# nlesc-dirac/sagecal

Hardware: NVIDIA H100
Metric: baseline_visibilities_per_sec_predict_jacobian (higher is better)
Workload: dtype f64

## Files before the change

sagecal_b200/csrc/lm.cu:

```cuda
#include <float.h>
#include <math.h>
#include <string.h>
#include <vector>

#include "../../include/dirac_b200.h"
#include "problem.h"

#define CS_CHECK(call)                                                                     \
  do {                                                                                     \
    cusolverStatus_t s__ = (call);                                                         \
    if (s__ != CUSOLVER_STATUS_SUCCESS) {                                                  \
      fprintf(stderr, "dirac_b200: cuSOLVER error %d at %s:%d\n", (int)s__, __FILE__, __LINE__); \
      exit(1);                                                                             \
    }                                                                                      \
  } while (0)
#define CB_CHECK(call)                                                                     \
  do {                                                                                     \
    cublasStatus_t s__ = (call);                                                           \
    if (s__ != CUBLAS_STATUS_SUCCESS) {                                                    \
      fprintf(stderr, "dirac_b200: cuBLAS error %d at %s:%d\n", (int)s__, __FILE__, __LINE__); \
      exit(1);                                                                             \
    }                                                                                      \
  } while (0)

extern "C" {
void db_launch_weighted_jtj(const WeightedJtjArgs *a, int ntile, cudaStream_t st);
void db_launch_sum_abs(const double2 *v, long long R, long long r0, long long r1, double *partials,
                       double *out, unsigned int *counter, cudaStream_t st);
void db_launch_update_weights(const double2 *e, double2 *wt, long long R, long long r0,
                              long long r1, double nu0, double *partials, double *out,
                              unsigned int *counter, cudaStream_t st);
void db_launch_scale_vis(double2 *v, long long R, long long r0, long long r1, double alpha,
                         int set_const, cudaStream_t st);
void db_launch_extract_diag(const double *A, double *dst, int n, cudaStream_t st);
void db_launch_lm_step(const double *p, const double *Dp, const double *jte, double *pnew,
                       double *sc, double *zero, int n, cudaStream_t st);
void db_launch_os_shift(const double2 *e, const double2 *wt, double2 *eps, double2 *wout, long long R,
                        long long row_sub0, long long nrow_sub, long long row_chunk0, long long kl,
                        long long nJ, cudaStream_t st);
}

template <typename T>
static T *dalloc(size_t n) {
  return (T *)db_malloc(n * sizeof(T) + 16);
}

void db_lm_init(dirac_b200_problem *pr) {
  LMWork &w = pr->lm;
  if (w.ready) return;
  DevProblem &d = pr->d;
  const int n8 = 8 * d.N;
  w.n8 = n8;
  w.T = dalloc<double>((size_t)d.Mt * d.Nbase * 16);
  w.T_valid = (unsigned char *)calloc(d.Mt, 1);
  w.Tsub = dalloc<double>((size_t)d.Nbase * 16);
  w.JTJ0 = dalloc<double>((size_t)n8 * n8);
  w.JTJ = dalloc<double>((size_t)n8 * n8);
  w.JTe = d.scal + 64 + n8;
  w.JTe_new = d.scal + 64 + 2 * n8;
  w.Hst = dalloc<double>((size_t)4 * d.N);
  w.Dp = d.scal + 64;
  w.pnew = dalloc<double>(n8);
  w.plast = dalloc<double>(n8);
  w.pold = dalloc<double>(n8);
  w.devinfo = reinterpret_cast<int *>(d.scal + 64 + 3 * n8);
  w.tau = dalloc<double>(n8);
  w.svdS = w.svdU = w.svdVT = nullptr;
  w.wbuf = w.ebuf = nullptr;
  w.os_eps = w.os_w = nullptr;
  w.HP = w.HQ = nullptr;
  w.JB = w.LB = nullptr;
  w.sys_T = w.sys_p = w.sys_H = nullptr;
  w.pref_slot = (int *)malloc(sizeof(int) * d.M);
  for (int k = 0; k < d.M; k++) w.pref_slot[k] = -1;
  w.jtj0_cur = nullptr;
  w.jtj_spec = nullptr;
  {
    const int nbg = (d.Nbase + 255) / 256;
    const int nsl = db_cp_max_slices(d.Nbase, d.tilesz);
    w.jte_part = dalloc<double>((size_t)nbg * (nsl + 1) * n8);
  }
  DB_CHECK(cudaEventCreateWithFlags(&w.ev_mail, cudaEventDisableTiming));
  DB_CHECK(cudaMallocHost((void **)&w.h_vec, sizeof(double) * (5 * n8 + 4 * d.N + 64)));
  static cusolverDnHandle_t g_cs = nullptr;
  static cublasHandle_t g_cb = nullptr;
  if (!g_cs) {
    CS_CHECK(cusolverDnCreate(&g_cs));
    CB_CHECK(cublasCreate(&g_cb));
  }
  w.cs = g_cs;
  w.cb = g_cb;
  CS_CHECK(cusolverDnSetStream(w.cs, d.stream));
  CB_CHECK(cublasSetStream(w.cb, d.stream));
  int l1 = 0, l2 = 0, l3 = 0;
  CS_CHECK(cusolverDnDpotrf_bufferSize(w.cs, CUBLAS_FILL_MODE_LOWER, n8, w.JTJ, n8, &l1));
  CS_CHECK(cusolverDnDgeqrf_bufferSize(w.cs, n8, n8, w.JTJ, n8, &l2));
  CS_CHECK(cusolverDnDormqr_bufferSize(w.cs, CUBLAS_SIDE_LEFT, CUBLAS_OP_T, n8, 1, n8, w.JTJ, n8,
                                       w.tau, w.Dp, n8, &l3));
  w.lwork = l1 > l2 ? l1 : l2;
  if (l3 > w.lwork) w.lwork = l3;
  int l4 = 0;
  CS_CHECK(cusolverDnDgesvd_bufferSize(w.cs, n8, n8, &l4));
  if (l4 > w.lwork) w.lwork = l4;
  w.own_chol = n8 <= db_chol_max_n() && db_chol_available() && !getenv("DIRAC_B200_CUSOLVER");
  if (w.own_chol && (size_t)w.lwork < db_chol_ws_doubles(n8)) w.lwork = (int)db_chol_ws_doubles(n8);
  w.cswork = dalloc<double>((size_t)w.lwork);
  w.bt_ws = nullptr;
  w.bt_epoch = 0;
  if (!w.own_chol && db_bigtri_available(n8)) {
    const size_t nd = db_bigtri_ws_doubles(n8);
    w.bt_ws = dalloc<double>(nd);
    DB_CHECK(cudaMemsetAsync(w.bt_ws, 0, sizeof(double) * nd, d.stream));
  }
  w.dbuf = dalloc<double2>((size_t)4 * d.R);
  w.ready = true;
}

static void robust_init(dirac_b200_problem *pr) {
  LMWork &w = pr->lm;
  if (w.wbuf) return;
  DevProblem &d = pr->d;
  w.wbuf = dalloc<double2>((size_t)4 * d.R);
  w.ebuf = dalloc<double2>((size_t)4 * d.R);
  w.HP = dalloc<double>((size_t)d.N * 20);
  w.HQ = dalloc<double>((size_t)d.N * 20);
}

static void os_init(dirac_b200_problem *pr) {
  robust_init(pr);
  LMWork &w = pr->lm;
  if (w.os_eps) return;
  w.os_eps = dalloc<double2>((size_t)4 * pr->d.R);
  w.os_w = dalloc<double2>((size_t)4 * pr->d.R);
}

void db_lm_free(dirac_b200_problem *pr) {
  LMWork &w = pr->lm;
  if (!w.ready) return;
  db_free(w.T); db_free(w.Tsub); db_free(w.JTJ0); db_free(w.JTJ);
  db_free(w.Hst); db_free(w.pnew); db_free(w.plast); db_free(w.pold); db_free(w.jte_part);
  db_free(w.tau); db_free(w.cswork); db_free(w.dbuf);
  if (w.bt_ws) db_free(w.bt_ws);
  if (w.svdS) { db_free(w.svdS); db_free(w.svdU); db_free(w.svdVT); }
  if (w.wbuf) { db_free(w.wbuf); db_free(w.ebuf); db_free(w.HP); db_free(w.HQ); }
  if (w.os_eps) { db_free(w.os_eps); db_free(w.os_w); }
  if (w.LB) {
    if (w.JB) db_free(w.JB);
    db_free(w.LB); db_free(w.HB); db_free(w.mu_dev); db_free(w.binfo_dev);
    db_free(w.LBptr_dev); db_free(w.blist_dev); db_free(w.btix_dev); db_free(w.bpoff_dev);
    cudaFreeHost(w.h_mu); cudaFreeHost(w.h_binfo);
  }
  free(w.pref_slot);
  cudaEventDestroy(w.ev_mail);
  cudaFreeHost(w.h_vec);
  free(w.T_valid);
  w.ready = false;
}

static int pick_tslice(const DevProblem &d, int nt) {
  int target_ctas = db_sm_count();
  int slices = (target_ctas + d.ntile - 1) / d.ntile;
  if (slices < 1) slices = 1;
  int ts = (nt + slices - 1) / slices;
  if (ts < 2) ts = 2;
  if (ts > nt) ts = nt;
  if (ts < 1) ts = 1;
  return ts;
}

void db_cluster_pass(dirac_b200_problem *pr, int k, const double *pblk_dev, const double2 *in,
                     double2 *out, int mode, int write_out, double *jte_dev, int cost_slot, int t0,
                     int t1, const double2 *wt, double beta = 1.0, const double2 *in2 = nullptr,
                     bool jte_zeroed = false, const double *pblk_old = nullptr,
                     bool form_hidden = false);

void db_cluster_pass(dirac_b200_problem *pr, int k, const double *pblk_dev, const double2 *in,
                     double2 *out, int mode, int write_out, double *jte_dev, int cost_slot, int t0,
                     int t1, const double2 *wt, double beta, const double2 *in2, bool jte_zeroed,
                     const double *pblk_old, bool form_hidden) {
  DevProblem &d = pr->d;
  if (t1 <= t0) {
    if (mode <= 1 || mode == 4)
      DB_CHECK(cudaMemsetAsync(d.scal + cost_slot, 0, sizeof(double), d.stream));
    if (jte_dev) DB_CHECK(cudaMemsetAsync(jte_dev, 0, sizeof(double) * 8 * d.N, d.stream));
    return;
  }
  ClusterPassArgs a;
  a.coh_k = d.coh + (size_t)k * 4 * d.R;
  a.in = in; a.flag = d.flag; a.pblk = pblk_dev; a.tiles = d.tiles; a.out = out; a.jte = jte_dev;
  a.blpq = d.blpq; a.jte_part = pr->lm.jte_part; a.gcounter = d.counters + 16;
  a.partials = pr->partials; a.cost = d.scal + cost_slot; a.counter = d.counters; a.R = d.R;
  a.N = d.N; a.Nbase = d.Nbase; a.t_begin = t0; a.t_end = t1; a.tslice = pick_tslice(d, t1 - t0);
  a.mode = mode; a.write_out = write_out; a.wt = wt; a.beta = beta; a.in2 = in2;
  a.pblk_old = pblk_old; a.form_hidden = form_hidden;
  if (!(jte_dev && (mode <= 1 || mode == 4)) && a.tslice > 1)
    a.tslice = (a.tslice + 1) / 2;
  if (jte_dev && (mode <= 1 || mode == 4) && !jte_zeroed)
    DB_CHECK(cudaMemsetAsync(jte_dev, 0, sizeof(double) * 8 * d.N, d.stream));
  db_prof_begin((jte_dev && (mode <= 1 || mode == 4)) ? 2 : 8, (double)(t1 - t0) * d.Nbase * (129.0 + (write_out ? 64.0 : 0.0) +
                                                 (wt ? 64.0 : 0.0)), d.stream);
  db_launch_cluster_pass(&a, d.ntile, d.stream);
  db_prof_end(d.stream);
  db_count_launch(1);
}

static void gram(dirac_b200_problem *pr, int k, int t0, int t1, int step, double *Tdst) {
  DevProblem &d = pr->d;
  GramArgs a;
  a.coh = d.coh; a.flag = d.flag; a.tiles = d.tiles; a.T = Tdst; a.R = d.R; a.N = d.N;
  a.Nbase = d.Nbase; a.k0 = k; a.t_begin = t0; a.t_end = t1; a.t_step = step;
  db_prof_begin(3, (double)((t1 - t0 + step - 1) / step) * d.Nbase * 65.0 + 128.0 * d.Nbase,
                d.stream);
  db_launch_coh_gram(&a, d.ntile, 1, d.stream);
  db_prof_end(d.stream);
  db_count_launch(1);
}

static AssembleArgs assemble_args(const DevProblem &d, const double *T, const double *pblk_dev,
                                  double *Hst) {
  AssembleArgs a;
  memset(&a, 0, sizeof(a));
  a.T = T; a.pblk = pblk_dev; a.Hst = Hst; a.N = d.N; a.Nbase = d.Nbase;
  return a;
}

static void station_sums(dirac_b200_problem *pr, const AssembleArgs &a, int nb) {
  DevProblem &d = pr->d;
  db_prof_begin(4, nb * 256.0 * d.Nbase, d.stream);
  db_launch_station_sums(&a, nb, d.stream);
  db_prof_end(d.stream);
  db_count_launch(1);
}

static void assemble_tiles(dirac_b200_problem *pr, const AssembleArgs &a, int nb) {
  DevProblem &d = pr->d;
  const double n = 8.0 * d.N;
  db_prof_begin(4, nb * (a.lower ? 128.0 * d.Nbase + 4.0 * n * (n + 1) : 256.0 * d.Nbase + 8.0 * n * n),
                d.stream);
  db_launch_assemble_tiles(&a, nb, d.stream);
  db_prof_end(d.stream);
  db_count_launch(1);
}

static void assemble(dirac_b200_problem *pr, const double *T, const double *pblk_dev,
                     double *JTJ) {
  AssembleArgs a = assemble_args(pr->d, T, pblk_dev, pr->lm.Hst);
  station_sums(pr, a, 1);
  if (!JTJ) return;
  a.JTJ = JTJ;
  assemble_tiles(pr, a, 1);
}

static void weighted_jtj(dirac_b200_problem *pr, int k, int t0, int t1, const double *pblk_dev,
                         const double2 *wt, double *JTJ) {
  DevProblem &d = pr->d;
  LMWork &w = pr->lm;
  const int n = w.n8;
  DB_CHECK(cudaMemsetAsync(JTJ, 0, sizeof(double) * (size_t)n * n, d.stream));
  DB_CHECK(cudaMemsetAsync(w.HP, 0, sizeof(double) * 20 * d.N, d.stream));
  DB_CHECK(cudaMemsetAsync(w.HQ, 0, sizeof(double) * 20 * d.N, d.stream));
  if (t1 <= t0) return;
  WeightedJtjArgs a;
  a.coh_k = d.coh + (size_t)k * 4 * d.R;
  a.wt = wt; a.flag = d.flag; a.pblk = pblk_dev; a.tiles = d.tiles; a.JTJ = JTJ; a.HP = w.HP;
  a.HQ = w.HQ; a.R = d.R; a.N = d.N; a.Nbase = d.Nbase; a.t_begin = t0; a.t_end = t1;
  a.tslice = pick_tslice(d, t1 - t0);
  db_prof_begin(6, (double)(t1 - t0) * d.Nbase * 129.0 + 8.0 * 64.0 * d.N * d.N, d.stream);
  db_launch_weighted_jtj(&a, d.ntile, d.stream);
  db_prof_end(d.stream);
  db_count_launch(2);
}

void db_chunk_range(const DevProblem &d, int k, int ck, int *t0, int *t1);
static void chunk_range(const DevProblem &d, int k, int ck, int *t0, int *t1) {
  db_chunk_range(d, k, ck, t0, t1);
}
void db_chunk_range(const DevProblem &d, int k, int ck, int *t0, int *t1) {
  int nchunk = d.h_clus[k].nchunk;
  int tilechunk = (d.tilesz + nchunk - 1) / nchunk;
  int a = ck * tilechunk;
  int b = a + tilechunk;
  if (a > d.tilesz) a = d.tilesz;
  if (b > d.tilesz) b = d.tilesz;
  *t0 = a;
  *t1 = b;
}

static int enqueue_solve(dirac_b200_problem *pr, double mu, int linsolv, double eps1) {
  DevProblem &d = pr->d;
  LMWork &w = pr->lm;
  const int n = w.n8;
  int *hinfo = (int *)(w.h_vec + 4 * n + 4 * d.N);
  hinfo[0] = hinfo[1] = 0;
  if (linsolv == 0 && w.own_chol) {
    db_prof_begin(5, 0.0, d.stream);
    db_launch_chol_solve(w.jtj0_cur ? w.jtj0_cur : w.JTJ0, n, mu, w.JTe, w.Dp, w.cswork, w.devinfo,
                         d.stream);
    db_prof_end(d.stream);
    db_count_launch(1);
    w.step_fused = w.step_armed;
    return 1;
  }
  if (linsolv == 0 && w.sys_T) {
    AssembleArgs a = assemble_args(d, w.sys_T, w.sys_p, const_cast<double *>(w.sys_H));
    a.JTJ = w.JTJ;
    a.mu = mu;
    a.lower = 1;
    assemble_tiles(pr, a, 1);
  } else {
    db_prof_begin(4, 16.0 * n * n, d.stream);
    db_launch_copy_add_diag(w.jtj0_cur ? w.jtj0_cur : w.JTJ0, w.JTJ, n, mu, d.stream);
    db_prof_end(d.stream);
    db_count_launch(1);
  }
  DB_CHECK(cudaMemcpyAsync(w.Dp, w.JTe, sizeof(double) * n, cudaMemcpyDeviceToDevice, d.stream));
  db_prof_begin(5, 0.0, d.stream);
  if (linsolv == 0) {
    CS_CHECK(cusolverDnDpotrf(w.cs, CUBLAS_FILL_MODE_LOWER, n, w.JTJ, n, w.cswork, w.lwork,
                              w.devinfo));
    if (w.bt_ws) {
      DB_CHECK(cudaMemsetAsync(w.devinfo + 1, 0, sizeof(int), d.stream));
      db_launch_bigtri_solve(w.JTJ, n, n, w.JTe, w.Dp, w.bt_ws, ++w.bt_epoch, 1, d.stream);
      db_count_launch(4);
    } else {
      CS_CHECK(cusolverDnDpotrs(w.cs, CUBLAS_FILL_MODE_LOWER, n, 1, w.JTJ, n, w.Dp, n,
                                w.devinfo + 1));
      db_count_launch(2);
    }
  } else if (linsolv == 1) {
    CS_CHECK(cusolverDnDgeqrf(w.cs, n, n, w.JTJ, n, w.tau, w.cswork, w.lwork, w.devinfo));
    CS_CHECK(cusolverDnDormqr(w.cs, CUBLAS_SIDE_LEFT, CUBLAS_OP_T, n, 1, n, w.JTJ, n, w.tau, w.Dp,
                              n, w.cswork, w.lwork, w.devinfo + 1));
    const double one = 1.0;
    CB_CHECK(cublasDtrsm(w.cb, CUBLAS_SIDE_LEFT, CUBLAS_FILL_MODE_UPPER, CUBLAS_OP_N,
                         CUBLAS_DIAG_NON_UNIT, n, 1, &one, w.JTJ, n, w.Dp, n));
    db_count_launch(3);
  } else {
    if (!w.svdS) {
      w.svdS = dalloc<double>(n);
      w.svdU = dalloc<double>((size_t)n * n);
      w.svdVT = dalloc<double>((size_t)n * n);
    }
    CS_CHECK(cusolverDnDgesvd(w.cs, 'A', 'A', n, n, w.JTJ, n, w.svdS, w.svdU, n, w.svdVT, n,
                              w.cswork, w.lwork, nullptr, w.devinfo));
    db_count_launch(1);
    double *hS = (double *)malloc(sizeof(double) * n);
    double *hb = (double *)malloc(sizeof(double) * n);
    const double one = 1.0, zero = 0.0;
    CB_CHECK(cublasDgemv(w.cb, CUBLAS_OP_T, n, n, &one, w.svdU, n, w.JTe, 1, &zero, w.Dp, 1));
    DB_CHECK(cudaMemcpyAsync(hS, w.svdS, sizeof(double) * n, cudaMemcpyDeviceToHost, d.stream));
    DB_CHECK(cudaMemcpyAsync(hb, w.Dp, sizeof(double) * n, cudaMemcpyDeviceToHost, d.stream));
    db_stream_sync(d.stream);
    for (int i = 0; i < n; i++) hb[i] = (hS[i] > eps1) ? hb[i] / hS[i] : 0.0;
    DB_CHECK(cudaMemcpyAsync(w.pnew, hb, sizeof(double) * n, cudaMemcpyHostToDevice, d.stream));
    CB_CHECK(cublasDgemv(w.cb, CUBLAS_OP_T, n, n, &one, w.svdVT, n, w.pnew, 1, &zero, w.Dp, 1));
    db_prof_end(d.stream);
    DB_CHECK(cudaMemcpyAsync(w.h_vec + 2 * n, w.Dp, sizeof(double) * n, cudaMemcpyDeviceToHost,
                             d.stream));
    db_stream_sync(d.stream);
    free(hS);
    free(hb);
    db_count_launch(2);
    return 1;
  }
  db_prof_end(d.stream);
  (void)hinfo;
  return 1;
}

static double nrm2sq(const double *v, int n) {
  double s = 0.0;
  for (int i = 0; i < n; i++) s += v[i] * v[i];
  return s;
}

void db_prefactor_sweep(dirac_b200_problem *pr, double tau) {
  DevProblem &d = pr->d;
  db_lm_init(pr);
  LMWork &w = pr->lm;
  const int n = w.n8;
  const size_t nn = (size_t)n * n;
  const bool own_batch = w.own_chol && db_tri_available(n) && !getenv("DIRAC_B200_BATCH_CUSOLVER");
  const bool keep_jb = w.own_chol;
  if ((double)d.M * nn * 8.0 * (keep_jb ? 2 : 1) > 24e9) return;
  const size_t lstride = own_batch ? db_chol_ws_doubles(n) : nn;
  w.lb_stride = lstride;
  w.lb_ld = own_batch ? 32 * ((n + 31) / 32) : n;
  if (!w.LB) {
    w.JB = keep_jb ? dalloc<double>(nn * d.M) : nullptr;
    w.LB = dalloc<double>(lstride * d.M);
    w.HB = dalloc<double>((size_t)4 * d.N * d.M);
    w.mu_dev = dalloc<double>(d.M);
    w.binfo_dev = dalloc<int>(2 * d.M);
    w.LBptr_dev = (double **)dalloc<double *>(d.M);
    w.blist_dev = dalloc<int>(d.M);
    w.btix_dev = dalloc<int>(d.M);
    w.bpoff_dev = dalloc<int>(d.M);
    DB_CHECK(cudaMallocHost((void **)&w.h_mu, sizeof(double) * d.M));
    DB_CHECK(cudaMallocHost((void **)&w.h_binfo, sizeof(int) * 2 * d.M));
    std::vector<int> tix(d.M), poff(d.M);
    std::vector<double *> ptr(d.M);
    for (int k = 0; k < d.M; k++) {
      tix[k] = d.h_clus[k].chunk0;
      poff[k] = d.h_chunk_poff[d.h_clus[k].chunk0];
      ptr[k] = w.LB + lstride * k;
    }
    DB_CHECK(cudaMemcpy(w.btix_dev, tix.data(), sizeof(int) * d.M, cudaMemcpyHostToDevice));
    DB_CHECK(cudaMemcpy(w.bpoff_dev, poff.data(), sizeof(int) * d.M, cudaMemcpyHostToDevice));
    DB_CHECK(cudaMemcpy(w.LBptr_dev, ptr.data(), sizeof(double *) * d.M, cudaMemcpyHostToDevice));
  }
  std::vector<int> list;
  for (int k = 0; k < d.M;) {
    const int tix = d.h_clus[k].chunk0;
    if (d.h_clus[k].nchunk != 1 || w.T_valid[tix]) {
      k++;
      continue;
    }
    int k1 = k + 1;
    while (k1 < d.M && d.h_clus[k1].nchunk == 1 && !w.T_valid[d.h_clus[k1].chunk0] &&
           d.h_clus[k1].chunk0 == tix + (k1 - k))
      k1++;
    GramArgs a;
    a.coh = d.coh; a.flag = d.flag; a.tiles = d.tiles; a.T = w.T + (size_t)tix * d.Nbase * 16;
    a.R = d.R; a.N = d.N; a.Nbase = d.Nbase; a.k0 = k; a.t_begin = 0; a.t_end = d.tilesz;
    a.t_step = 1;
    db_prof_begin(3, (double)(k1 - k) * ((double)d.tilesz * d.Nbase * 65.0 + 128.0 * d.Nbase),
                  d.stream);
    db_launch_coh_gram(&a, d.ntile, k1 - k, d.stream);
    db_prof_end(d.stream);
    db_count_launch(1);
    for (int kk = k; kk < k1; kk++) w.T_valid[d.h_clus[kk].chunk0] = 1;
    k = k1;
  }
  for (int k = 0; k < d.M; k++) {
    w.pref_slot[k] = -1;
    if (d.h_clus[k].nchunk != 1) continue;
    w.pref_slot[k] = (int)list.size();
    list.push_back(k);
  }
  const int nb = (int)list.size();
  if (nb == 0) return;
  DB_CHECK(cudaMemcpyAsync(w.blist_dev, list.data(), sizeof(int) * nb, cudaMemcpyHostToDevice,
                           d.stream));
  AssembleArgs b = assemble_args(d, w.T, d.pp, w.HB);
  b.list = w.blist_dev; b.tix = w.btix_dev; b.poff = w.bpoff_dev;
  station_sums(pr, b, nb);
  db_launch_batch_mu0(w.HB, w.mu_dev, d.N, tau, nb, d.stream);
  db_count_launch(1);
  if (keep_jb) {
    b.JTJ = w.JB;
    b.stride = (long long)nn;
    assemble_tiles(pr, b, nb);
  }
  if (!own_batch) {
    b.JTJ = w.LB;
    b.stride = (long long)lstride;
    b.mu_dev = w.mu_dev;
    b.lower = 1;
    assemble_tiles(pr, b, nb);
  }
  db_prof_begin(5, 0.0, d.stream);
  if (own_batch) {
    db_launch_chol_factor_batched(w.JB, n, w.mu_dev, w.LB, (long long)lstride, w.binfo_dev, nb,
                                  d.stream);
    db_count_launch(1);
  } else if (n <= 1024) {
    CS_CHECK(cusolverDnDpotrfBatched(w.cs, CUBLAS_FILL_MODE_LOWER, n, w.LBptr_dev, n, w.binfo_dev, nb));
    db_count_launch(1);
  } else {
    enum { NS = 4 };
    static cudaStream_t fs[NS];
    static cusolverDnHandle_t fh[NS];
    static double *fwork[NS];
    static int flwork = 0;
    static cudaEvent_t fev[NS], fstart;
    if (!flwork || flwork < w.lwork) {
      for (int i = 0; i < NS; i++) {
        if (!flwork) {
          DB_CHECK(cudaStreamCreateWithFlags(&fs[i], cudaStreamNonBlocking));
          CS_CHECK(cusolverDnCreate(&fh[i]));
          CS_CHECK(cusolverDnSetStream(fh[i], fs[i]));
          DB_CHECK(cudaEventCreateWithFlags(&fev[i], cudaEventDisableTiming));
        } else {
          db_free(fwork[i]);
        }
        fwork[i] = dalloc<double>((size_t)w.lwork);
      }
      if (!flwork) DB_CHECK(cudaEventCreateWithFlags(&fstart, cudaEventDisableTiming));
      flwork = w.lwork;
    }
    DB_CHECK(cudaEventRecord(fstart, d.stream));
    for (int i = 0; i < NS && i < nb; i++) DB_CHECK(cudaStreamWaitEvent(fs[i], fstart, 0));
    for (int b = 0; b < nb; b++) {
      const int i = b % NS;
      CS_CHECK(cusolverDnDpotrf(fh[i], CUBLAS_FILL_MODE_LOWER, n, w.LB + nn * b, n, fwork[i], flwork,
                                w.binfo_dev + b));
    }
    for (int i = 0; i < NS && i < nb; i++) {
      DB_CHECK(cudaEventRecord(fev[i], fs[i]));
      DB_CHECK(cudaStreamWaitEvent(d.stream, fev[i], 0));
    }
    db_count_launch(nb);
  }
  db_prof_end(d.stream);
  DB_CHECK(cudaMemcpyAsync(w.h_mu, w.mu_dev, sizeof(double) * nb, cudaMemcpyDeviceToHost, d.stream));
  DB_CHECK(cudaMemcpyAsync(w.h_binfo, w.binfo_dev, sizeof(int) * (own_batch ? 2 * nb : nb),
                           cudaMemcpyDeviceToHost, d.stream));
  w.binfo_step = own_batch ? 2 : 1;
  db_stream_sync(d.stream);
}

static long g_noise_decisions = 0;
static long g_lm_stat[4] = {0, 0, 0, 0};
extern "C" void dirac_b200_lm_stats(long *out4, int reset) {
  for (int i = 0; i < 4; i++) {
    if (out4) out4[i] = g_lm_stat[i];
    if (reset) g_lm_stat[i] = 0;
  }
}
extern "C" long dirac_b200_noise_decisions(int reset) {
  const long v = g_noise_decisions;
  if (reset) g_noise_decisions = 0;
  return v;
}

struct LmAug {
  const double *y_dev, *bz_dev;
  const double *y_host, *bz_host;
  double rho;
};
static const LmAug *g_aug = nullptr;
static std::vector<double> g_hpnew;
static double *hpnew_aug(LMWork &w) {
  if ((int)g_hpnew.size() < w.n8) g_hpnew.resize(w.n8);
  return g_hpnew.data();
}
static double aug_cost(const LmAug *a, const double *p, int n) {
  double s = 0.0;
  for (int i = 0; i < n; i++) {
    const double dlt = p[i] - a->bz_host[i];
    s += a->y_host[i] * dlt + 0.5 * a->rho * dlt * dlt;
  }
  return s;
}
extern "C" void db_launch_lm_aug_rhs(double *jte, const double *p, const double *y, const double *bz,
                                     double rho, int n, cudaStream_t st);

struct LmOut {
  double init_eL2, eL2, jacTe_inf, Dp_L2, mu;
  int k, stop;
  bool res_in_dbuf;
};

struct OsLayout {
  int Nsubsets, Ntper;
  bool misaligned;
};
static OsLayout os_layout(int ntiles) {
  OsLayout o;
  o.Nsubsets = ntiles < 10 ? ntiles : 10;
  o.Ntper = o.Nsubsets > 0 ? (ntiles + o.Nsubsets - 1) / o.Nsubsets : ntiles;
  o.misaligned = o.Nsubsets > 0 && (ntiles % o.Nsubsets) != 0 && !db_opt(DB_OPT_OS_CONSISTENT);
  return o;
}

struct OsPath {
  bool misaligned;
  int s0, s1;
  long long nJ;
};

static OsPath os_subset_system(dirac_b200_problem *pr, int k, int t0, int t1, int l,
                               const double *pblk_dev, const double2 *wt) {
  DevProblem &d = pr->d;
  LMWork &w = pr->lm;
  const int ntiles = t1 - t0;
  const OsLayout L = os_layout(ntiles);
  const int Ntper = L.Ntper;
  OsPath path;
  path.misaligned = L.misaligned;
  path.nJ = 0;
  int s0 = t0 + l * Ntper;
  int s1 = (l * Ntper + Ntper < ntiles) ? s0 + Ntper : t1;
  if (s0 > t1) s0 = t1;
  if (!L.misaligned) {
    db_cluster_pass(pr, k, pblk_dev, w.dbuf, nullptr, 1, 0, w.JTe, 2, s0, s1, wt);
    if (wt) {
      weighted_jtj(pr, k, s0, s1, pblk_dev, wt, w.JTJ0);
    } else {
      gram(pr, k, s0, s1, 1, w.Tsub);
      assemble(pr, w.Tsub, pblk_dev, w.JTJ0);
    }
  } else {
    const long long nn = 8ll * ntiles * d.Nbase;
    const long long Nper = (nn + L.Nsubsets - 1) / L.Nsubsets;
    const long long kl = (long long)l * Nper;
    const int tl = l * Ntper;
    long long Nos;
    int tileI;
    if (tl + Ntper < ntiles) {
      Nos = Nper;
      tileI = Ntper;
    } else {
      Nos = nn - kl;
      tileI = ntiles - tl;
    }
    long long nJ = tileI > 0 ? 8ll * d.Nbase * tileI : 0;
    if (Nos < nJ) nJ = Nos;
    if (nJ < 0) nJ = 0;
    s0 = t0 + tl;
    s1 = s0 + (tileI > 0 ? tileI : 0);
    if (s0 > t1) s0 = s1 = t1;
    os_init(pr);
    db_cluster_pass(pr, k, pblk_dev, w.dbuf, w.ebuf, 1, 1, nullptr, 2, t0, t1, nullptr);
    if (s1 > s0) {
      db_launch_os_shift(w.ebuf, wt, w.os_eps, w.os_w, d.R, (long long)s0 * d.Nbase,
                         (long long)(s1 - s0) * d.Nbase, (long long)t0 * d.Nbase, kl, nJ, d.stream);
      db_count_launch(1);
    }
    db_cluster_pass(pr, k, pblk_dev, w.os_eps, nullptr, 4, 0, w.JTe, 2, s0, s1, w.os_w);
    weighted_jtj(pr, k, s0, s1, pblk_dev, w.os_w, w.JTJ0);
    path.nJ = nJ;
  }
  path.s0 = s0;
  path.s1 = s1;
  return path;
}

static void lm_core(dirac_b200_problem *pr, int k, int ck, int t0, int t1, double *pblk_dev,
                    const double2 *wt, int itmax, const double *opts, int linsolv, int os,
                    int os_shift, int randomize, bool have_first, double first_cost, int *nu_damp,
                    bool *evaluated_trial, const double2 *hidden_from, LmOut *out) {
  DevProblem &d = pr->d;
  LMWork &w = pr->lm;
  const int n = w.n8;
  const int ntiles = t1 - t0;
  const double tau = opts[0], eps1 = opts[1], eps2 = opts[2], eps2_sq = opts[2] * opts[2],
               eps3 = opts[3];
  double *hp = w.h_vec;
  double *hjte = w.h_vec + n;
  double *hDp = w.h_vec + 2 * n;
  double *hpnew = w.h_vec + 3 * n;
  double *hH = w.h_vec + 4 * n;

  double p_eL2;
  const LmAug *aug = (!os && !wt) ? g_aug : nullptr;
  const double half_rho = aug ? 0.5 * aug->rho : 0.0;
  if (aug) w.pref_slot[k] = -1;
  const bool defer = have_first && !os && !wt && linsolv == 0 && itmax > 0 && w.pref_slot[k] >= 0 &&
                     std::isnan(first_cost);
  DB_CHECK(cudaMemcpyAsync(hp, pblk_dev, sizeof(double) * n, cudaMemcpyDeviceToHost, d.stream));
  if (aug && have_first)
    db_launch_lm_aug_rhs(w.JTe, pblk_dev, aug->y_dev, aug->bz_dev, aug->rho, n, d.stream);
  if (have_first) {
    p_eL2 = first_cost;
// ... 722 lines not shown
```

sagecal_b200/csrc/problem.h:

```cpp
#pragma once
#include <cusolverDn.h>
#include <cublas_v2.h>

#include <vector>

#include "../../include/dirac_b200.h"
#include "internal.cuh"

struct LMWork {
  bool ready;
  int n8;
  double *T;
  unsigned char *T_valid;
  double *Tsub;
  double *JTJ0, *JTJ;
  double *JTe, *JTe_new;
  double *Hst;
  double *Dp;
  double *pnew;
  double *h_vec;
  int *devinfo;
  double *cswork;
  int lwork;
  bool own_chol;
  double *bt_ws;
  unsigned bt_epoch;
  double *jte_part;
  bool step_armed, step_fused;
  double *jtj_spec;
  cudaEvent_t ev_mail;
  double *tau;
  double *svdS, *svdU, *svdVT;
  cusolverDnHandle_t cs;
  cublasHandle_t cb;
  double2 *dbuf;
  double2 *wbuf;
  double2 *ebuf;
  double2 *os_eps, *os_w;
  double *HP, *HQ;
  double *plast;
  double *pold;
  double *JB, *LB;
  size_t lb_stride;
  int lb_ld, binfo_step;
  double *HB;
  double *mu_dev;
  double *h_mu;
  int *binfo_dev, *h_binfo;
  double **LBptr_dev;
  int *blist_dev, *btix_dev, *bpoff_dev;
  int *pref_slot;
  const double *jtj0_cur;
  const double *sys_T, *sys_p, *sys_H;
};

struct dirac_b200_problem {
  DevProblem d;
  double *partials;
  int npartials;
  double2 *res;
  double2 *vis_stage;
  double *g;
  LMWork lm;
  int own_stream;
  int rank, world;
  void (*allreduce)(void *dev, long long count, void *stream, void *user);
  void *comm_user;
  int m_global;
  int k_global0;
  double beta;
  const double *aug_y_host, *aug_bz_host, *aug_rho;
  double *aug_dev;
  double2 *pm;
  double *xb;
  double *pp_start;
  double2 *E0, *E1, *E2;
  struct RtrWork *rtr;
};

void db_stream_sync(cudaStream_t st);
void db_event_sync(cudaEvent_t ev);
void db_flag_wait(const volatile unsigned long long *flag, unsigned long long epoch,
                  cudaStream_t st);
void *db_malloc(size_t bytes);
void db_free(void *p);
void require_gpu();

class DeviceScope {
 public:
  DeviceScope();
  explicit DeviceScope(cudaStream_t borrowed);
  ~DeviceScope();
  DeviceScope(const DeviceScope &) = delete;
  DeviceScope &operator=(const DeviceScope &) = delete;
  template <class T> T *alloc(size_t n) {
    void *p = nullptr;
    DB_CHECK(cudaMalloc(&p, sizeof(T) * n));
    bufs_.push_back(p);
    return (T *)p;
  }
  template <class T> T *upload(const T *h, size_t n) {
    T *d = alloc<T>(n ? n : 1);
    if (n) DB_CHECK(cudaMemcpyAsync(d, h, sizeof(T) * n, cudaMemcpyHostToDevice, st));
    return d;
  }
  template <class T> T *upload(const std::vector<T> &h) { return upload(h.data(), h.size()); }
  void sync();
  const cudaStream_t st;

 private:
  const bool own_;
  std::vector<void *> bufs_;
};

void db_download_coh(const double2 *coh, double *x, int M, long long R, cudaStream_t st);
void db_count_launch(int n);
void db_prof_begin(int kind, double bytes, cudaStream_t st);
void db_prof_end(cudaStream_t st);
cudaStream_t db_new_stream(int *owned);
void db_upload_vis(dirac_b200_problem *pr, const double *h, double2 *dst);
void db_download_vis(dirac_b200_problem *pr, const double2 *src, double *h);
void db_predict_dev(dirac_b200_problem *pr, const double *pp_dev, double2 *out, int out_mode,
                    int cost_mode, double nu, int slot);
double db_read_scalar(dirac_b200_problem *pr, int slot);
void db_grad_dev(dirac_b200_problem *pr, const double *pp_dev, double *g_dev, int robust,
                 double nu);
double db_cost_window_dev(dirac_b200_problem *pr, const double *pp_dev, double2 *out, double nu,
                          long long r_lo, long long r_hi);
void db_grad_window_dev(dirac_b200_problem *pr, const double *pp_dev, double *g_dev, double nu,
                        long long r_lo, long long r_hi);
int db_bfgsfit_dev(dirac_b200_problem *pr, double *pp, int max_lbfgs, int lbfgs_m, int solver_mode,
                   double mean_nu, double *res_0, double *res_1, bool keep_residual);
void db_count_sky_upload();
void db_count_coh_host_bytes(size_t bytes);
void db_lm_init(dirac_b200_problem *pr);
void db_prefactor_sweep(dirac_b200_problem *pr, double tau);
void db_allreduce(dirac_b200_problem *pr, void *dev, long long count);
void db_allreduce_world(dirac_b200_problem *pr, void *dev, long long count);
void db_lm_set_aug(const double *y_dev, const double *bz_dev, const double *y_host,
                   const double *bz_host, double rho);
int db_overlap_available(const dirac_b200_problem *pr);
cudaStream_t db_comm_stream();
void db_allreduce_segments(dirac_b200_problem *pr, double **ptr, const long long *count, int nseg,
                           cudaStream_t st);
extern "C" {
void db_launch_residual_cost(const double2 *x, const double2 *pm, double2 *out, long long n4,
                             int out_mode, int cost_mode, double inv_nu, double *partials,
                             double *cost, unsigned int *counter, cudaStream_t st);
void db_launch_axpby(const double2 *x, double2 *y, long long n4, double a, double b,
                     cudaStream_t st);
void db_launch_cluster_rowmap(const double2 *coh_k, const double2 *in, const double2 *in2,
                              double2 *out, const unsigned char *flag, const double *pp,
                              const int *chunk_poff, int nchunk, const short2 *blpq, long long R,
                              int Nbase, int sign, double beta, cudaStream_t st);
}

struct BandView {
  const double2 *coh, *x;
  const unsigned char *flag;
  int nc;
};
struct BandDev {
  int N, Nbase, tilesz, M, Mt, maxnc, ntile;
  long long R, npar;
  ClusterDesc *clus;
  int *chunk_poff;
  TileDesc *tiles;
  short2 *blpq;
  double *pp, *g, *partials, *scal, *h_scal;
  unsigned int *counters;
  double2 *res;
  cudaStream_t st;
};
void db_build_tiles(int N, std::vector<TileDesc> &tiles);
void db_canonical_flags(int N, int Nbase, int tilesz, const baseline_t *barr, unsigned char *flag);
BandDev *db_band_create(int N, int Nbase, int tilesz, const clus_source_t *carr, int M, int Mt,
                        int maxnc, cudaStream_t st);
void db_band_destroy(BandDev *bd);
void db_band_fit(BandDev *bd, const BandView &b, double *p, const double *y, const double *z,
// ... 8 lines not shown
```

Measured before the change: 6.655 billion.

## Replace per-matrix multi-stream dpotrf with batched blocked Cholesky using lookahead

For large per-cluster normal matrices (n>1024) that do not use the custom Cholesky, the code now uses a blocked right-looking batched factorization. Each panel is factored with batched potrf and inverted via trsm+gemm, trailing updates run as strided-batched GEMMs, and the next panel overlaps with the trailing update on a side stream. This replaces looping cusolverDnDpotrf over four streams. It adds many more launches and extra workspace, and only affects the LM block-factor path, not the predict/Jacobian throughput metric. A standalone benchmark script and entry point are also added.

Measured after the change: 6.987 billion (median of 6 runs). 1.05x the previous value.

```diff
diff --git a/profiles/big_factor.py b/profiles/big_factor.py
--- /dev/null
+++ b/profiles/big_factor.py
@@ -0,0 +1,41 @@
+import argparse
+import ctypes as C
+import json
+import os
+import sys
+
+ROOT = os.path.dirname(os.path.dirname(os.path.abspath(__file__)))
+sys.path.insert(0, ROOT)
+sys.path.insert(0, os.path.dirname(os.path.abspath(__file__)))
+from sagecal_b200 import lib as blib
+from minibatch_stage import card
+
+VARIANTS = ["dpotrf", "dpotrf_4_streams", "blocked_trsm", "blocked_inv", "blocked_inv_lookahead"]
+
+
+def main():
+    ap = argparse.ArgumentParser()
+    ap.add_argument("--n", type=int, default=4096)
+    ap.add_argument("--batch", type=int, default=32)
+    ap.add_argument("--reps", type=int, default=3)
+    args = ap.parse_args()
+    L = blib.load().lib
+    L.dirac_b200_bench_big_factor.restype = C.c_int
+    L.dirac_b200_bench_big_factor.argtypes = [C.c_int, C.c_int, C.c_int, C.c_int, C.POINTER(C.c_double)]
+    rep = {"n": args.n, "batch": args.batch, "reps": args.reps}
+    rep["card"], rep["power_limit_and_max_sm_clock"] = card()
+    gflop = args.n ** 3 / 3.0 * 1e-9
+    for batch in sorted({1, args.batch}):
+        for v, name in enumerate(VARIANTS):
+            us = (C.c_double * 4)()
+            bad = L.dirac_b200_bench_big_factor(args.n, batch, args.reps, v, us)
+            per = us[0] / batch
+            r = {"us_per_factor": round(per, 1), "tflops": round(gflop / per * 1e3, 2), "bad_status": bad}
+            if v in (2, 3):
+                r["us_panels_trailing_per_factor"] = [round(us[i] / batch, 1) for i in (1, 2)]
+            rep["%s_x%d" % (name, batch)] = r
+    print(json.dumps(rep))
+
+
+if __name__ == "__main__":
+    main()
diff --git a/sagecal_b200/csrc/bigchol.cu b/sagecal_b200/csrc/bigchol.cu
--- /dev/null
+++ b/sagecal_b200/csrc/bigchol.cu
@@ -0,0 +1,360 @@
+#include <vector>
+
+#include "problem.h"
+
+#define BC_CS(call)                                                                        \
+  do {                                                                                     \
+    cusolverStatus_t s__ = (call);                                                         \
+    if (s__ != CUSOLVER_STATUS_SUCCESS) {                                                  \
+      fprintf(stderr, "dirac_b200: cuSOLVER error %d at %s:%d\n", (int)s__, __FILE__, __LINE__); \
+      exit(1);                                                                             \
+    }                                                                                      \
+  } while (0)
+#define BC_CB(call)                                                                        \
+  do {                                                                                     \
+    cublasStatus_t s__ = (call);                                                           \
+    if (s__ != CUBLAS_STATUS_SUCCESS) {                                                    \
+      fprintf(stderr, "dirac_b200: cuBLAS error %d at %s:%d\n", (int)s__, __FILE__, __LINE__); \
+      exit(1);                                                                             \
+    }                                                                                      \
+  } while (0)
+
+
+struct BigChol {
+  int n, nbk, np;
+  int maxb;
+  double *A0;
+  long long stride;
+  double **ptr;
+  int *pinfo;
+  bool inv_panel;
+  double *X, *W;
+  double **Xptr;
+  bool lookahead;
+};
+
+namespace {
+
+struct Lib {
+  cublasHandle_t cb[2];
+  cusolverDnHandle_t cs[2];
+  cudaStream_t side;
+  cudaEvent_t ev_main, ev_side;
+};
+Lib &lib() {
+  static Lib L;
+  static bool made = false;
+  if (!made) {
+    for (int i = 0; i < 2; i++) {
+      BC_CB(cublasCreate(&L.cb[i]));
+      BC_CS(cusolverDnCreate(&L.cs[i]));
+    }
+    DB_CHECK(cudaStreamCreateWithFlags(&L.side, cudaStreamNonBlocking));
+    DB_CHECK(cudaEventCreateWithFlags(&L.ev_main, cudaEventDisableTiming));
+    DB_CHECK(cudaEventCreateWithFlags(&L.ev_side, cudaEventDisableTiming));
+    BC_CB(cublasSetStream(L.cb[1], L.side));
+    BC_CS(cusolverDnSetStream(L.cs[1], L.side));
+    made = true;
+  }
+  return L;
+}
+
+inline int width(int n, int nbk, int j) { return (n - j * nbk) < nbk ? n - j * nbk : nbk; }
+
+__global__ void k_bigchol_info(const int *pinfo, int np, int nbk, int ld, int nb, int *info,
+                               int info_step) {
+  const int b = blockIdx.x * blockDim.x + threadIdx.x;
+  if (b >= nb) return;
+  int v = 0;
+  for (int j = 0; j < np; j++) {
+    const int l = pinfo[(size_t)j * ld + b];
+    if (l != 0) {
+      v = l > 0 ? j * nbk + l : l;
+      break;
+    }
+  }
+  info[(size_t)b * info_step] = v;
+}
+
+void trailing(cublasHandle_t cb, double *A, long long stride, int nb, int n, int nbk, int j, int c0,
+              int c1) {
+  const double mone = -1.0, one = 1.0;
+  const int wj = width(n, nbk, j);
+  for (int c = c0; c < c1; c++) {
+    const int r = c * nbk, m = n - r;
+    const double *Lc = A + (size_t)j * nbk * n + r;
+    double *C = A + (size_t)r * n + r;
+    BC_CB(cublasDgemmStridedBatched(cb, CUBLAS_OP_N, CUBLAS_OP_T, m, width(n, nbk, c), wj, &mone, Lc, n,
+                                    stride, Lc, n, stride, &one, C, n, stride, nb));
+  }
+}
+
+__global__ void k_bigchol_eye(double *X, int w, long long stride, int nb) {
+  const long long ww = (long long)w * w;
+  for (long long t = blockIdx.x * (long long)blockDim.x + threadIdx.x; t < ww * nb;
+       t += (long long)gridDim.x * blockDim.x) {
+    const long long e = t % ww;
+    X[(t / ww) * stride + e] = (e % w == e / w) ? 1.0 : 0.0;
+  }
+}
+
+__global__ void k_bigchol_put(const double *src, long long sstride, double *dst, long long dstride,
+                              int ld, int m, int w, int nb) {
+  const long long mw = (long long)m * w;
+  for (long long t = blockIdx.x * (long long)blockDim.x + threadIdx.x; t < mw * nb;
+       t += (long long)gridDim.x * blockDim.x) {
+    const long long b = t / mw, e = t - b * mw;
+    const long long off = (e / m) * ld + e % m;
+    dst[b * dstride + off] = src[b * sstride + off];
+  }
+}
+
+}
+
+BigChol *db_bigchol_create(int n, int nbk, bool inv_panel, bool lookahead) {
+  lib();
+  BigChol *bc = new BigChol();
+  bc->n = n;
+  bc->nbk = nbk;
+  bc->np = (n + nbk - 1) / nbk;
+  bc->maxb = 0;
+  bc->A0 = nullptr;
+  bc->stride = 0;
+  bc->ptr = nullptr;
+  bc->pinfo = nullptr;
+  bc->inv_panel = inv_panel;
+  bc->lookahead = lookahead;
+  bc->X = bc->W = nullptr;
+  bc->Xptr = nullptr;
+  return bc;
+}
+
+void db_bigchol_bind_batch(BigChol *bc, double *A0, long long stride, int maxb) {
+  if (bc->A0 == A0 && bc->stride == stride && bc->maxb >= maxb) return;
+  const int n = bc->n, nbk = bc->nbk, np = bc->np;
+  std::vector<double *> h((size_t)2 * np * maxb);
+  for (int j = 0; j < np; j++) {
+    const int r = j * nbk;
+    for (int b = 0; b < maxb; b++) {
+      double *Ajj = A0 + stride * b + (size_t)r * n + r;
+      h[(size_t)(2 * j) * maxb + b] = Ajj;
+      h[(size_t)(2 * j + 1) * maxb + b] = Ajj + width(n, nbk, j);
+    }
+  }
+  if (bc->ptr) db_free(bc->ptr);
+  if (bc->pinfo) db_free(bc->pinfo);
+  bc->ptr = (double **)db_malloc(sizeof(double *) * h.size());
+  bc->pinfo = (int *)db_malloc(sizeof(int) * (size_t)np * maxb);
+  DB_CHECK(cudaMemcpy(bc->ptr, h.data(), sizeof(double *) * h.size(), cudaMemcpyHostToDevice));
+  if (bc->inv_panel) {
+    if (bc->X) { db_free(bc->X); db_free(bc->W); db_free(bc->Xptr); }
+    bc->X = (double *)db_malloc(sizeof(double) * nbk * nbk * maxb);
+    bc->W = (double *)db_malloc(sizeof(double) * (size_t)nbk * n * maxb);
+    std::vector<double *> xp(maxb);
+    for (int b = 0; b < maxb; b++) xp[b] = bc->X + (size_t)nbk * nbk * b;
+    bc->Xptr = (double **)db_malloc(sizeof(double *) * maxb);
+    DB_CHECK(cudaMemcpy(bc->Xptr, xp.data(), sizeof(double *) * maxb, cudaMemcpyHostToDevice));
+  }
+  bc->A0 = A0;
+  bc->stride = stride;
+  bc->maxb = maxb;
+}
+
+void db_bigchol_destroy(BigChol *bc) {
+  if (!bc) return;
+  if (bc->ptr) db_free(bc->ptr);
+  if (bc->pinfo) db_free(bc->pinfo);
+  if (bc->X) { db_free(bc->X); db_free(bc->W); db_free(bc->Xptr); }
+  delete bc;
+}
+
+static void panel(BigChol *bc, int nb, int j, cublasHandle_t cb, cusolverDnHandle_t cs, cudaStream_t st) {
+  const int n = bc->n, nbk = bc->nbk, mb = bc->maxb;
+  const int wj = width(n, nbk, j), m = n - j * nbk - wj;
+  const double one = 1.0;
+  BC_CS(cusolverDnDpotrfBatched(cs, CUBLAS_FILL_MODE_LOWER, wj, bc->ptr + (size_t)2 * j * mb, n,
+                                bc->pinfo + (size_t)j * mb, nb));
+  if (m > 0 && bc->inv_panel) {
+    const double zero = 0.0;
+    const long long xs = (long long)nbk * nbk, ws = (long long)nbk * n;
+    double *Aij = bc->A0 + (size_t)j * nbk * n + j * nbk + wj;
+    k_bigchol_eye<<<2 * db_sm_count(), 256, 0, st>>>(bc->X, wj, xs, nb);
+    BC_CB(cublasDtrsmBatched(cb, CUBLAS_SIDE_LEFT, CUBLAS_FILL_MODE_LOWER, CUBLAS_OP_N,
+                             CUBLAS_DIAG_NON_UNIT, wj, wj, &one, bc->ptr + (size_t)2 * j * mb, n,
+                             bc->Xptr, wj, nb));
+    BC_CB(cublasDgemmStridedBatched(cb, CUBLAS_OP_N, CUBLAS_OP_T, m, wj, wj, &one, Aij, n, bc->stride,
+                                    bc->X, wj, xs, &zero, bc->W, n, ws, nb));
+    k_bigchol_put<<<4 * db_sm_count(), 256, 0, st>>>(bc->W, ws, Aij, bc->stride, n, m, wj, nb);
+  } else if (m > 0) {
+    BC_CB(cublasDtrsmBatched(cb, CUBLAS_SIDE_RIGHT, CUBLAS_FILL_MODE_LOWER, CUBLAS_OP_T,
+                             CUBLAS_DIAG_NON_UNIT, m, wj, &one, bc->ptr + (size_t)2 * j * mb, n,
+                             bc->ptr + (size_t)(2 * j + 1) * mb, n, nb));
+  }
+}
+
+static void factor_batch(BigChol *bc, int nb, int *info, int info_step, cudaStream_t st,
+                         double *phase_ms) {
+  Lib &L = lib();
+  const int n = bc->n, nbk = bc->nbk, np = bc->np, mb = bc->maxb;
+  BC_CB(cublasSetStream(L.cb[0], st));
+  BC_CS(cusolverDnSetStream(L.cs[0], st));
+  if (bc->lookahead) {
+    panel(bc, nb, 0, L.cb[0], L.cs[0], st);
+    for (int j = 0; j + 1 < np; j++) {
+      trailing(L.cb[0], bc->A0, bc->stride, nb, n, nbk, j, j + 1, j + 2);
+      DB_CHECK(cudaEventRecord(L.ev_main, st));
+      DB_CHECK(cudaStreamWaitEvent(L.side, L.ev_main, 0));
+      panel(bc, nb, j + 1, L.cb[1], L.cs[1], L.side);
+      DB_CHECK(cudaEventRecord(L.ev_side, L.side));
+      trailing(L.cb[0], bc->A0, bc->stride, nb, n, nbk, j, j + 2, np);
+      DB_CHECK(cudaStreamWaitEvent(st, L.ev_side, 0));
+    }
+  } else {
+    cudaEvent_t ev[3];
+    if (phase_ms)
+      for (int i = 0; i < 3; i++) DB_CHECK(cudaEventCreate(&ev[i]));
+    for (int j = 0; j < np; j++) {
+      if (phase_ms) DB_CHECK(cudaEventRecord(ev[0], st));
+      panel(bc, nb, j, L.cb[0], L.cs[0], st);
+      if (phase_ms) DB_CHECK(cudaEventRecord(ev[1], st));
+      trailing(L.cb[0], bc->A0, bc->stride, nb, n, nbk, j, j + 1, np);
+      if (phase_ms) {
+        DB_CHECK(cudaEventRecord(ev[2], st));
+        DB_CHECK(cudaEventSynchronize(ev[2]));
+        for (int i = 0; i < 2; i++) {
+          float ms = 0.f;
+          DB_CHECK(cudaEventElapsedTime(&ms, ev[i], ev[i + 1]));
+          phase_ms[i] += ms;
+        }
+      }
+    }
+    if (phase_ms)
+      for (int i = 0; i < 3; i++) cudaEventDestroy(ev[i]);
+  }
+  k_bigchol_info<<<(nb + 127) / 128, 128, 0, st>>>(bc->pinfo, np, nbk, mb, nb, info, info_step);
+  db_count_launch((bc->inv_panel ? 5 : 2) * np + np * (np - 1) / 2 + 1);
+}
+
+void db_bigchol_factor_batch(BigChol *bc, int nb, int *info, int info_step, cudaStream_t st) {
+  factor_batch(bc, nb, info, info_step, st, nullptr);
+}
+
+namespace {
+__global__ void k_bigchol_fill(double *A, int n, long long stride, int nb) {
+  const long long nn = (long long)n * n;
+  for (long long t = blockIdx.x * (long long)blockDim.x + threadIdx.x; t < nn * nb;
+       t += (long long)gridDim.x * blockDim.x) {
+    const int b = (int)(t / nn);
+    const long long e = t - (long long)b * nn;
+    const int i = (int)(e % n), jj = (int)(e / n);
+    double v = 1.0 / (1.0 + fabs((double)(i - jj)) + b);
+    if (i == jj) v += n;
+    A[(size_t)b * stride + e] = v;
+  }
+}
+}
+
+extern "C" {
+int dirac_b200_big_factor(int n, int nb, double *A, int *info) {
+  if (n <= 512 || nb < 1) return -1;
+  const size_t nn = (size_t)n * n;
+  double *dA = (double *)db_malloc(sizeof(double) * nn * nb);
+  int *dinfo = (int *)db_malloc(sizeof(int) * nb);
+  DB_CHECK(cudaMemcpy(dA, A, sizeof(double) * nn * nb, cudaMemcpyHostToDevice));
+  cudaStream_t st;
+  DB_CHECK(cudaStreamCreateWithFlags(&st, cudaStreamNonBlocking));
+  BigChol *bc = db_bigchol_create(n, BC_BLOCK, BC_INV_PANEL, BC_LOOKAHEAD);
+  db_bigchol_bind_batch(bc, dA, (long long)nn, nb);
+  db_bigchol_factor_batch(bc, nb, dinfo, 1, st);
+  DB_CHECK(cudaStreamSynchronize(st));
+  DB_CHECK(cudaMemcpy(A, dA, sizeof(double) * nn * nb, cudaMemcpyDeviceToHost));
+  DB_CHECK(cudaMemcpy(info, dinfo, sizeof(int) * nb, cudaMemcpyDeviceToHost));
+  db_bigchol_destroy(bc);
+  cudaStreamDestroy(st);
+  db_free(dA);
+  db_free(dinfo);
+  DB_CHECK(cudaGetLastError());
+  return 0;
+}
+
+int dirac_b200_bench_big_factor(int n, int batch, int reps, int variant, double *us_out) {
+  if (n <= 512 || batch < 1 || reps < 1 || variant < 0 || variant > 4) return -1;
+  const size_t nn = (size_t)n * n;
+  double *dA = (double *)db_malloc(sizeof(double) * nn * batch);
+  int *dinfo = (int *)db_malloc(sizeof(int) * batch);
+  cudaStream_t st;
+  DB_CHECK(cudaStreamCreateWithFlags(&st, cudaStreamNonBlocking));
+  enum { NS = 4 };
+  cudaStream_t fs[NS];
+  cusolverDnHandle_t fh[NS];
+  cudaEvent_t fev[NS], e0, e1;
+  double *fwork[NS];
+  int lw = 0;
+  {
+    cusolverDnHandle_t h;
+    BC_CS(cusolverDnCreate(&h));
+    BC_CS(cusolverDnDpotrf_bufferSize(h, CUBLAS_FILL_MODE_LOWER, n, dA, n, &lw));
+    cusolverDnDestroy(h);
+  }
+  for (int i = 0; i < NS; i++) {
+    DB_CHECK(cudaStreamCreateWithFlags(&fs[i], cudaStreamNonBlocking));
+    BC_CS(cusolverDnCreate(&fh[i]));
+    BC_CS(cusolverDnSetStream(fh[i], fs[i]));
+    DB_CHECK(cudaEventCreateWithFlags(&fev[i], cudaEventDisableTiming));
+    fwork[i] = (double *)db_malloc(sizeof(double) * (lw > 1 ? lw : 1));
+  }
+  DB_CHECK(cudaEventCreate(&e0));
+  DB_CHECK(cudaEventCreate(&e1));
+  BigChol *bc = db_bigchol_create(n, BC_BLOCK, variant >= 3, variant == 4);
+  db_bigchol_bind_batch(bc, dA, (long long)nn, batch);
+  double total_ms = 0.0;
+  int bad = 0;
+  std::vector<int> h(batch);
+  for (int r = 0; r < reps + 1; r++) {
+    k_bigchol_fill<<<4 * db_sm_count(), 256, 0, st>>>(dA, n, (long long)nn, batch);
+    DB_CHECK(cudaEventRecord(e0, st));
+    if (variant == 0 || variant == 1) {
+      const int ns = variant == 0 ? 1 : NS;
+      for (int i = 0; i < ns; i++) DB_CHECK(cudaStreamWaitEvent(fs[i], e0, 0));
+      for (int b = 0; b < batch; b++)
+        BC_CS(cusolverDnDpotrf(fh[b % ns], CUBLAS_FILL_MODE_LOWER, n, dA + nn * b, n, fwork[b % ns],
+                               lw, dinfo + b));
+      for (int i = 0; i < ns; i++) {
+        DB_CHECK(cudaEventRecord(fev[i], fs[i]));
+        DB_CHECK(cudaStreamWaitEvent(st, fev[i], 0));
+      }
+    } else {
+      db_bigchol_factor_batch(bc, batch, dinfo, 1, st);
+    }
+    DB_CHECK(cudaEventRecord(e1, st));
+    DB_CHECK(cudaEventSynchronize(e1));
+    float ms = 0.f;
+    DB_CHECK(cudaEventElapsedTime(&ms, e0, e1));
+    if (r > 0) total_ms += ms;
+    DB_CHECK(cudaMemcpy(h.data(), dinfo, sizeof(int) * batch, cudaMemcpyDeviceToHost));
+    for (int b = 0; b < batch; b++) bad += h[b] != 0;
+  }
+  us_out[0] = 1e3 * total_ms / reps;
+  if (variant == 2 || variant == 3) {
+    double ph[2] = {0.0, 0.0};
+    k_bigchol_fill<<<4 * db_sm_count(), 256, 0, st>>>(dA, n, (long long)nn, batch);
+    factor_batch(bc, batch, dinfo, 1, st, ph);
+    DB_CHECK(cudaStreamSynchronize(st));
+    for (int i = 0; i < 2; i++) us_out[1 + i] = 1e3 * ph[i];
+  }
+  db_bigchol_destroy(bc);
+  for (int i = 0; i < NS; i++) {
+    cusolverDnDestroy(fh[i]);
+    cudaStreamDestroy(fs[i]);
+    cudaEventDestroy(fev[i]);
+    db_free(fwork[i]);
+  }
+  cudaEventDestroy(e0);
+  cudaEventDestroy(e1);
+  cudaStreamDestroy(st);
+  db_free(dA);
+  db_free(dinfo);
+  DB_CHECK(cudaGetLastError());
+  return bad;
+}
+}
diff --git a/sagecal_b200/csrc/lm.cu b/sagecal_b200/csrc/lm.cu
--- a/sagecal_b200/csrc/lm.cu
+++ b/sagecal_b200/csrc/lm.cu
@@ -105,6 +105,7 @@
   w.own_chol = n8 <= db_chol_max_n() && db_chol_available() && !getenv("DIRAC_B200_CUSOLVER");
   if (w.own_chol && (size_t)w.lwork < db_chol_ws_doubles(n8)) w.lwork = (int)db_chol_ws_doubles(n8);
   w.cswork = dalloc<double>((size_t)w.lwork);
+  w.bc = (!w.own_chol && n8 > 1024) ? db_bigchol_create(n8, BC_BLOCK, BC_INV_PANEL, BC_LOOKAHEAD) : nullptr;
   w.bt_ws = nullptr;
   w.bt_epoch = 0;
   if (!w.own_chol && db_bigtri_available(n8)) {
@@ -141,6 +142,7 @@
   db_free(w.Hst); db_free(w.pnew); db_free(w.plast); db_free(w.pold); db_free(w.jte_part);
   db_free(w.tau); db_free(w.cswork); db_free(w.dbuf);
   if (w.bt_ws) db_free(w.bt_ws);
+  db_bigchol_destroy(w.bc);
   if (w.svdS) { db_free(w.svdS); db_free(w.svdU); db_free(w.svdVT); }
   if (w.wbuf) { db_free(w.wbuf); db_free(w.ebuf); db_free(w.HP); db_free(w.HQ); }
   if (w.os_eps) { db_free(w.os_eps); db_free(w.os_w); }
@@ -408,6 +410,7 @@
     DB_CHECK(cudaMemcpy(w.btix_dev, tix.data(), sizeof(int) * d.M, cudaMemcpyHostToDevice));
     DB_CHECK(cudaMemcpy(w.bpoff_dev, poff.data(), sizeof(int) * d.M, cudaMemcpyHostToDevice));
     DB_CHECK(cudaMemcpy(w.LBptr_dev, ptr.data(), sizeof(double *) * d.M, cudaMemcpyHostToDevice));
+    if (w.bc) db_bigchol_bind_batch(w.bc, w.LB, (long long)lstride, d.M);
   }
   std::vector<int> list;
   for (int k = 0; k < d.M;) {
@@ -464,43 +467,11 @@
     db_launch_chol_factor_batched(w.JB, n, w.mu_dev, w.LB, (long long)lstride, w.binfo_dev, nb,
                                   d.stream);
     db_count_launch(1);
-  } else if (n <= 1024) {
+  } else if (!w.bc) {
     CS_CHECK(cusolverDnDpotrfBatched(w.cs, CUBLAS_FILL_MODE_LOWER, n, w.LBptr_dev, n, w.binfo_dev, nb));
     db_count_launch(1);
   } else {
-    enum { NS = 4 };
-    static cudaStream_t fs[NS];
-    static cusolverDnHandle_t fh[NS];
-    static double *fwork[NS];
-    static int flwork = 0;
-    static cudaEvent_t fev[NS], fstart;
-    if (!flwork || flwork < w.lwork) {
-      for (int i = 0; i < NS; i++) {
-        if (!flwork) {
-          DB_CHECK(cudaStreamCreateWithFlags(&fs[i], cudaStreamNonBlocking));
-          CS_CHECK(cusolverDnCreate(&fh[i]));
-          CS_CHECK(cusolverDnSetStream(fh[i], fs[i]));
-          DB_CHECK(cudaEventCreateWithFlags(&fev[i], cudaEventDisableTiming));
-        } else {
-          db_free(fwork[i]);
-        }
-        fwork[i] = dalloc<double>((size_t)w.lwork);
-      }
-      if (!flwork) DB_CHECK(cudaEventCreateWithFlags(&fstart, cudaEventDisableTiming));
-      flwork = w.lwork;
-    }
-    DB_CHECK(cudaEventRecord(fstart, d.stream));
-    for (int i = 0; i < NS && i < nb; i++) DB_CHECK(cudaStreamWaitEvent(fs[i], fstart, 0));
-    for (int b = 0; b < nb; b++) {
-      const int i = b % NS;
-      CS_CHECK(cusolverDnDpotrf(fh[i], CUBLAS_FILL_MODE_LOWER, n, w.LB + nn * b, n, fwork[i], flwork,
-                                w.binfo_dev + b));
-    }
-    for (int i = 0; i < NS && i < nb; i++) {
-      DB_CHECK(cudaEventRecord(fev[i], fs[i]));
-      DB_CHECK(cudaStreamWaitEvent(d.stream, fev[i], 0));
-    }
-    db_count_launch(nb);
+    db_bigchol_factor_batch(w.bc, nb, w.binfo_dev, 1, d.stream);
   }
   db_prof_end(d.stream);
   DB_CHECK(cudaMemcpyAsync(w.h_mu, w.mu_dev, sizeof(double) * nb, cudaMemcpyDeviceToHost, d.stream));
diff --git a/sagecal_b200/csrc/problem.h b/sagecal_b200/csrc/problem.h
--- a/sagecal_b200/csrc/problem.h
+++ b/sagecal_b200/csrc/problem.h
@@ -6,6 +6,14 @@
 
 #include "../../include/dirac_b200.h"
 #include "internal.cuh"
+
+struct BigChol;
+BigChol *db_bigchol_create(int n, int nbk, bool inv_panel, bool lookahead);
+enum { BC_BLOCK = 256 };
+static const bool BC_INV_PANEL = true, BC_LOOKAHEAD = true;
+void db_bigchol_destroy(BigChol *bc);
+void db_bigchol_bind_batch(BigChol *bc, double *A0, long long stride, int maxb);
+void db_bigchol_factor_batch(BigChol *bc, int nb, int *info, int info_step, cudaStream_t st);
 
 struct LMWork {
   bool ready;
@@ -25,6 +33,7 @@
   bool own_chol;
   double *bt_ws;
   unsigned bt_epoch;
+  BigChol *bc;
   double *jte_part;
   bool step_armed, step_fused;
   double *jtj_spec;
```
